# bjack205/rsLQR

Measured on AMD Instinct MI355X. Metric: LQR solves/sec (nx=12,nu=4,N=256,batch=1024 per GPU), higher is better.
Workload: dtype f64; 1 GPU; nx=12 nu=4 N=256 batch=1024 per GPU, fp64, factor+solve per step; parallelism=batch-sharded x1, no data-path collective, ranks_seen=1, flags=0, schedule=reduced-fused2

## Files before the change

### include/ndlqr_hip.h

```cpp
#ifndef NDLQR_HIP_H_
#define NDLQR_HIP_H_

#include <stddef.h>
#include <stdint.h>

#ifdef __cplusplus
extern "C" {
#endif

typedef struct NdlqrHipCtx NdlqrHipCtx;

int ndlqr_hip_device_count(void);
const char* ndlqr_hip_last_error(void);

NdlqrHipCtx* ndlqr_hip_create(int nstates, int ninputs, int nhorizon, int batch, int device);
#define NDLQR_CREATE_NO_PAD 1u
NdlqrHipCtx* ndlqr_hip_create_ex(int nstates, int ninputs, int nhorizon, int batch, int device, unsigned create_flags);
void ndlqr_hip_destroy(NdlqrHipCtx* ctx);
int ndlqr_hip_set_flags(NdlqrHipCtx* ctx, unsigned flags);
unsigned ndlqr_hip_get_flags(const NdlqrHipCtx* ctx);
int ndlqr_hip_set_stream(NdlqrHipCtx* ctx, void* hip_stream);
void* ndlqr_hip_get_stream(NdlqrHipCtx* ctx);

int ndlqr_hip_upload_inputs(NdlqrHipCtx* ctx, int p0, int count, const double* AB,
// ... 114 lines not shown
void ndlqr_hip_device_free(void* p);
int ndlqr_hip_copy(void* dst, const void* src, size_t bytes);

int ndlqr_hip_download_solutions(NdlqrHipCtx* ctx, int p0, int count, double* soln);
int ndlqr_hip_download_rhs_blocks(NdlqrHipCtx* ctx, int p, double* z_full);
int ndlqr_hip_download_factors(NdlqrHipCtx* ctx, int p, double* fact);
int ndlqr_hip_factors_valid(const NdlqrHipCtx* ctx);
int ndlqr_hip_pack_solutions_device(NdlqrHipCtx* ctx, double* dst);
int ndlqr_hip_kkt_residual(NdlqrHipCtx* ctx, double* res, double* bnorm);
int ndlqr_hip_cholesky_failures(NdlqrHipCtx* ctx);
int ndlqr_hip_download_failure_counts(NdlqrHipCtx* ctx, int* counts);
const char* ndlqr_hip_schedule(const NdlqrHipCtx* ctx);
int ndlqr_hip_compact_level1(const NdlqrHipCtx* ctx);
int ndlqr_hip_level1_paired(const NdlqrHipCtx* ctx);
int ndlqr_hip_bottom_lds16(const NdlqrHipCtx* ctx);

int ndlqr_hip_profile_slots(NdlqrHipCtx* ctx);
int ndlqr_hip_profile_get(NdlqrHipCtx* ctx, int slot, char* name, int name_cap, double* total_ms,
                          int* launches);
int ndlqr_hip_profile_reset(NdlqrHipCtx* ctx);

int ndlqr_hip_gemm(int tA, int tB, int m, int n, int k, double alpha, const double* A, int lda,
                   const double* B, int ldb, double beta, double* C, int ldc);
int ndlqr_hip_potrf_lower(int n, double* A, int lda);
int ndlqr_hip_potrs_lower(int n, int nrhs, const double* L, int ldl, double* B, int ldb);
int ndlqr_hip_trsv_lower(int n, int nrhs, const double* L, int ldl, double* B, int ldb, int transposed);

#ifdef __cplusplus
}
#endif
// ... 2 lines not shown
```

### rslqr_amd/__init__.py

```python
from .api import (
    BOUNDS_SHARED,
    BatchSolver,
    DeviceArray,
    FLAG_GENERIC,
    FLAG_KEEP_FACT,
    FLAG_KEEP_RECORDS,
    FLAG_PROFILE,
    FLAG_STRICT_FP,
    GRAD_A,
    GRAD_B,
    GRAD_DENSE_NAMES,
    GRAD_NAMES,
    GRAD_Q,
    GRAD_R,
    GRAD_d,
    GRAD_q,
    GRAD_r,
    GRAD_x0,
    GRADD_A,
    GRADD_B,
    GRADD_H,
    GRADD_Q,
    GRADD_R,
    GRADD_d,
# ... 8 lines not shown
    NdLqrBoxSettings,
    NdLqrBoxSettingsFull,
    NdLqrSolver,
    SOLN_INPUT,
    SOLN_ONLY,
    SOLN_LAMBDA,
    SOLN_STATE,
    device_count,
    exported_symbols,
    feedback_gains_lds,
    generate_synthetic,
    lib,
    library_path,
    objective_constants,
    pinned_empty,
)
```

### rslqr_amd/api.py

```python
import ctypes as C
import os
import re

import numpy as np

from . import build as _build

FLAG_STRICT_FP = 1
FLAG_GENERIC = 2
FLAG_PROFILE = 4
FLAG_KEEP_FACT = 8
FLAG_KEEP_RECORDS = 16
SOLN_LAMBDA, SOLN_STATE, SOLN_INPUT, SOLN_ONLY = 1, 2, 4, 8
GRAD_A, GRAD_B, GRAD_Q, GRAD_R, GRAD_q, GRAD_r, GRAD_d, GRAD_x0 = 1, 2, 4, 8, 16, 32, 64, 128
GRAD_NAMES = ("A", "B", "Q", "R", "q", "r", "d", "x0")
GRADD_A, GRADD_B, GRADD_Q, GRADD_H, GRADD_R, GRADD_q, GRADD_r, GRADD_d, GRADD_x0 = 1, 2, 4, 8, 16, 32, 64, 128, 256
GRAD_DENSE_NAMES = ("A", "B", "Q", "H", "R", "q", "r", "d", "x0")

ERR_INVALID = -1
ERR_NO_DEVICE = -2
ERR_NOT_SPD = -3

dp = C.POINTER(C.c_double)

# ... 308 lines not shown
    proto("ndlqr_hip_profile_slots", ci, vp)
    proto("ndlqr_hip_profile_get", ci, vp, ci, C.c_char_p, ci, dp, C.POINTER(ci))
    proto("ndlqr_hip_profile_reset", ci, vp)
    proto("ndlqr_hip_device_pointers", ci, vp, C.POINTER(vp))
    proto("ndlqr_hip_staged_io", ci, vp, C.POINTER(dp), C.POINTER(dp), C.POINTER(dp), C.POINTER(dp))
    proto("ndlqr_hip_download_rhs_blocks", ci, vp, ci, dp)
    proto("ndlqr_hip_upload_inputs", ci, vp, ci, ci, dp, dp, dp)
    proto("ndlqr_hip_factors_valid", ci, vp)
    proto("ndlqr_hip_schedule", C.c_char_p, vp)
    if hasattr(L, "ndlqr_hip_compact_level1"):
        proto("ndlqr_hip_compact_level1", C.c_int, vp)
    if hasattr(L, "ndlqr_hip_level1_paired"):
        proto("ndlqr_hip_level1_paired", C.c_int, vp)
    if hasattr(L, "ndlqr_hip_bottom_lds16"):
        proto("ndlqr_hip_bottom_lds16", C.c_int, vp)
    proto("ndlqr_hip_set_pipeline_depth", ci, vp, ci)
    proto("ndlqr_hip_pipeline_depth", ci, vp)
    proto("ndlqr_hip_pack_solutions_device", ci, vp, vp)
    proto("ndlqr_hip_gemm", ci, ci, ci, ci, ci, ci, cd, dp, ci, dp, ci, cd, dp, ci)
    proto("ndlqr_hip_potrf_lower", ci, ci, dp, ci)
    proto("ndlqr_hip_potrs_lower", ci, ci, ci, dp, ci, dp, ci)
    proto("ndlqr_hip_trsv_lower", ci, ci, ci, dp, ci, dp, ci, ci)
    _LIB = L
    return L


def pinned_empty(shape):
    import weakref
    count = int(np.prod(shape))
    L = lib()
# ... 110 lines not shown
        if not hasattr(a, "ptr"):
            if a.shape not in ((k,), (N, k), (B, N, k)):
                raise ValueError("bounds of shape %s: expected (%d,), (%d, %d) or (%d, %d, %d)" % (a.shape, k, N, k, B, N, k))
            a = np.ascontiguousarray(np.broadcast_to(a, (N, k) if shared else (B, N, k)))
            keep.append(a)
        ptrs.append(_any_ptr(a, (1 if shared else B) * N * k))
    return ptrs, shared, keep


def generate_synthetic(n, m, N, seed):
    out = dict(A=np.zeros((N, n * n)), B=np.zeros((N, n * m)), Q=np.zeros((N, n)),
               R=np.zeros((N, m)), q=np.zeros((N, n)), r=np.zeros((N, m)), d=np.zeros((N, n)),
               x0=np.zeros(n))
    _call(lib(), "ndlqr_GenerateSyntheticFlat", n, m, N, seed, *[_ptr(a) for a in out.values()], detail=False)
    return out


class BatchSolver:

    def __init__(self, n, m, N, batch, device=-1, flags=0):
        self.L = lib()
        self.n, self.m, self.N, self.batch = n, m, N, batch
        self.h = self.L.ndlqr_NewBatchSolver(n, m, N, batch, device)
        if not self.h:
            raise RuntimeError("ndlqr_NewBatchSolver failed: %s" %
                               self.L.ndlqr_hip_last_error().decode())
        self.nvars = self.L.ndlqr_BatchNumVars(self.h)
        self._sel = None
        self._step_refs = []
        self._rows = 0
# ... 589 lines not shown
```

### rslqr_amd/csrc/hip_context.hpp

```cpp
#pragma once
#include <hip/hip_runtime.h>

#include <cstdio>
#include <cstdlib>
#include <cstring>
#include <initializer_list>
#include <string>
#include <utility>
#include <vector>

#include "ndlqr.h"
#include "ndlqr_hip.h"

#include "kernels_common.hpp"

#pragma GCC visibility push(hidden)
int ndlqr_hip_fail(const char* what, hipError_t e);
struct NdlqrHipCtx;
int ndlqr_hip_ensure_F(NdlqrHipCtx* c);
#pragma GCC visibility pop
#define HIP_TRY(expr)                                                  \
  do {                                                                 \
    hipError_t e_ = (expr);                                            \
    if (e_ != hipSuccess) return ndlqr_hip_fail(#expr, e_);            \
// ... 15 lines not shown
  hipEvent_t start, stop;
};

enum class Family { None, Small, GenericReduced, GenericKnot };

struct KeptState {
  Family family = Family::None;
  bool time_shard = false;
  bool rec_complete = false;
  bool rec_compact = false;
  bool fact_valid = false;
  const char* schedule = "none";
  bool rec1_compact = false;
  bool level1_paired = false;
  bool bottom_lds16 = false;
  void forget_factorisation() { rec_complete = fact_valid = false; }
};

struct CapturedChain {
  hipGraphExec_t exec = nullptr;
  unsigned flags = 0;
  hipStream_t stream = nullptr;
  unsigned apply = 0;
  void reset() {
    if (exec) (void)hipGraphExecDestroy(exec);
    exec = nullptr;
  }
};

struct KnotSlice {
// ... 75 lines not shown
  unsigned long long rhs_gen[4] = {};
  CapturedChain graph;
  bool ready = false;
  hipError_t ensure_xfer(const ndlqr::Dims& u) { return xfer.ensure((size_t)u.batch * u.N * u.rows + (size_t)u.batch * u.n); }
};


struct DevKnobs {
  int rowbcast = -1;
  int tree = -1;
  int backsub_cols = -1;
  int fuse2 = -1;
  int compact1 = -1;
  int pair1 = -1;
  int bottom_lds16 = -1;
  int pipeline = 2;
  bool no_top = false;
  int top_levels = 3;
  bool no_mfma = false;
  int sep_threads = 0;
  int mult_threads = 0;
  bool no_reduced_generic = false;
  bool no_pad = false;
  bool alt_priority_set = false;
  int alt_priority = 0;
};

struct AdjointState {
  DevBuf<double> rhs, z;
  DevBuf<double> save;
  unsigned long long gen = 0;
  unsigned long long rhs_stamp = 0;
// ... 342 lines not shown
```

### rslqr_amd/csrc/kernels_bottom_reduced.hpp

```cpp
#pragma once
#include "kernels_dpp.hpp"
#include "kernels_small.hpp"

namespace ndlqr {

typedef double acc4_t __attribute__((ext_vector_type(4)));

template <int NX>
struct McPitch {
  static constexpr int SP = 18, WP = 17;
};

template <int NX, class Hook>
__device__ __forceinline__ void factor_tail_mc(const int lane, const acc4_t& c, const double (&ra)[(NX + 3) / 4],
                                               const double (&rb)[(NX + 3) / 4], const double* Wm, acc4_t& X0,
                                               acc4_t& X1, Hook hook) {
  constexpr int KS = (NX + 3) / 4, WP = McPitch<NX>::WP;
  int lane_o = lane;
  asm volatile("" : "+v"(lane_o));
  const int li = lane_o & 15, lk = lane_o >> 4;
  double wt[KS], wa[KS], b0[KS];
#pragma unroll
  for (int q = 0; q < KS; ++q) {
    wt[q] = Wm[(4 * q + lk) * WP + li];
// ... 867 lines not shown
      flag_failure(info, d, b);
  }
  __syncthreads();
  pair1_tail_park_mc<NX, NU>(d, kw + 4 * wave, b, lane, lds[wave].buf, hd, wave == 0, mslot, park);
  __syncthreads();
  asm volatile("" : "+v"(lane));
  if (wave == 0) reduced_eliminate_pass_mc<NX, NU>(d, kw, b, lane, c_m, mslot, info, lds[0].buf);
  __syncthreads();
  if (wave == 0) reduced_eliminate_gram_park_mc<NX, NU>(d, kw, b, lane, red, lds[0].buf, park);
  else reduced_eliminate_tail_mc<NX, NU>(d, kw, b, lane, false, red, rec, lds[0].buf);
}

template <int NX>
__device__ __forceinline__ void backsub_top_body(const Dims& d, const int b, const int t,
                                                 const double* __restrict__ recs, double* __restrict__ ytop,
                                                 double* ytop_lds, const int bp = -1, const double* zsep = nullptr);
template <int NX, int NU>
__global__ __launch_bounds__(256) __attribute__((amdgpu_waves_per_eu(4))) void reduced_top_mc(Dims d, const int l0, const double* __restrict__ AB,
                                                      const double* __restrict__ QR, const double* __restrict__ rhs,
                                                      double* red, double* __restrict__ rec, double* F,
                                                      int* __restrict__ info, const int store_l,
                                                      double* __restrict__ ytop) {
  __shared__ ReducedLds<NX, NU, false> lds[4];
  const int wave = __builtin_amdgcn_readfirstlane(threadIdx.x >> 6), b = blockIdx.x;
  for (int l = l0, s0 = 0; l < d.K;) {
    int lane = threadIdx.x & 63;
    asm volatile("" : "+v"(lane));
    const int cnt = d.N >> (l + 1);
    if (wave + s0 < cnt)
      reduced_separator_mc<NX, NU, true>(d, l, (wave + s0) * (2 << l), b, lane, AB, QR, rhs, red, rec, F, info, store_l,
                                         lds[wave]);
// ... 296 lines not shown
```

### rslqr_amd/csrc/kernels_rowbcast.hpp

```cpp
#pragma once
#include "kernels_dpp.hpp"
#include "kernels_small.hpp"

namespace ndlqr {

template <int K, bool NEG>
__device__ __forceinline__ void fmac_bc4(double& a0, double& a1, double& a2, double& a3, const double x0, const double x1,
                                         const double x2, const double x3, const double y) {
  if constexpr (NEG)
    asm volatile("v_fmac_f64_dpp %0, -%4, %8 row_newbcast:%9 row_mask:0xf bank_mask:0xf\n\t"
                 "v_fmac_f64_dpp %1, -%5, %8 row_newbcast:%9 row_mask:0xf bank_mask:0xf\n\t"
                 "v_fmac_f64_dpp %2, -%6, %8 row_newbcast:%9 row_mask:0xf bank_mask:0xf\n\t"
                 "v_fmac_f64_dpp %3, -%7, %8 row_newbcast:%9 row_mask:0xf bank_mask:0xf"
                 : "+v"(a0), "+v"(a1), "+v"(a2), "+v"(a3) : "v"(x0), "v"(x1), "v"(x2), "v"(x3), "v"(y), "n"(K));
  else
    asm volatile("v_fmac_f64_dpp %0, %4, %8 row_newbcast:%9 row_mask:0xf bank_mask:0xf\n\t"
                 "v_fmac_f64_dpp %1, %5, %8 row_newbcast:%9 row_mask:0xf bank_mask:0xf\n\t"
                 "v_fmac_f64_dpp %2, %6, %8 row_newbcast:%9 row_mask:0xf bank_mask:0xf\n\t"
                 "v_fmac_f64_dpp %3, %7, %8 row_newbcast:%9 row_mask:0xf bank_mask:0xf"
                 : "+v"(a0), "+v"(a1), "+v"(a2), "+v"(a3) : "v"(x0), "v"(x1), "v"(x2), "v"(x3), "v"(y), "n"(K));
}

template <int KD, int NC, bool INIT, bool NEG = false, int NA, int NB>
__device__ __forceinline__ void rb_mul(const double (&A)[NA], double (&B)[NB], double (&out)[NC]) {
// ... 338 lines not shown
    }
    rb_mul<NX, NX, true>(RbTt, Xb, G);
    gv = rb_mulv<NX>(RbTt, xz);
    if (hasB && rowlane) {
#pragma unroll
      for (int c = 0; c < NX; ++c)
        if (c >= i) atomicAdd(sB.DL() + c * (c + 1) / 2 + i, G[c]);
      atomicAdd(sB.gL() + i, gv);
    }
  }
}

template <int NX>
__device__ __forceinline__ void backsub_top_body(const Dims& d, const int b, const int t,
                                                 const double* __restrict__ recs, double* __restrict__ ytop,
                                                 double* ytop_lds, const int bp, const double* zsep) {
  constexpr int NN = NX * NX, REC = 2 * NN + NX;
  const int N = d.N, K = d.K;
  const int br = bp >= 0 ? bp : b;
  for (int L = K - 1; L >= 3; --L) {
    const int T = 2 << L, nsep = N >> (L + 1);
    for (int it = t; it < nsep * NX; it += 256) {
      const int q = it / NX, r = it - q * NX;
      const int base = q * T, s = base + (T >> 1) - 1;
      const double* rc = recs + ((size_t)br * N + s) * REC;
      double acc = zsep ? zsep[((size_t)b * N + s) * NX + r] : rc[2 * NN + r];
      if (base > 0) {
        double f[NX];
        load_row<NX>(rc + r * NX, f);
        const double* y = ytop_lds + ((base - 1) >> 3) * NX;
#pragma unroll
        for (int c = 0; c < NX; ++c) acc = fma(-f[c], y[c], acc);
      }
      if (base + T < N) {
        double f[NX];
        load_row<NX>(rc + NN + r * NX, f);
        const double* y = ytop_lds + ((base + T - 1) >> 3) * NX;
#pragma unroll
        for (int c = 0; c < NX; ++c) acc = fma(-f[c], y[c], acc);
      }
      ytop_lds[(s >> 3) * NX + r] = acc;
    }
    __syncthreads();
  }
  double* out = ytop + (size_t)b * (N >> 3) * NX;
  for (int e = t; e < ((N >> 3) - 1) * NX; e += 256) out[e] = ytop_lds[e];
}

template <int NX>
__global__ __launch_bounds__(256) void rb_backsub_top(Dims d, const double* __restrict__ recs, double* __restrict__ ytop) {
  extern __shared__ double ytop_lds[];
  backsub_top_body<NX>(d, blockIdx.x, threadIdx.x, recs, ytop, ytop_lds);
}

template <int NX, int NU>
struct alignas(16) RbBacksubLds {
  static constexpr int W = NX + NU, ROWS = 2 * NX + NU, NN = NX * NX, REC = 2 * NN + NX, R0 = NX * (NX + 1) / 2;
  static constexpr int R0P = (R0 + 1) / 2 * 2;
  static constexpr int WP = RbKnot<NX, NU>::WP;
  double ab[8][NX * WP];
  double rec0[4][R0P];
// ... 799 lines not shown
```

### rslqr_amd/csrc/launch_small.hpp

```cpp
#pragma once
#include "hip_context.hpp"
#include "kernels_leaf.hpp"
#include "kernels_small.hpp"
#include "kernels_bottom_reduced.hpp"
#include "kernels_rowbcast.hpp"

constexpr int kBottomLevels = 2;

struct SmallPlan {
  bool strict, keep;
  bool lean;
  int store_l;
  bool reduced;
  bool tree;
  bool compact;
  bool rowbcast;
  bool fuse2;
  bool compact1;
  bool pair1;
  bool lds16;
  int level0;
  int ltop;
  int top_l0;
  bool top_sweeps;
  size_t top_lds;
  const char* schedule;
  bool rec_complete, rec_compact;
  bool needs_F;
};

template <int NX, int NU>
constexpr bool kRbBacksubFits = 8 * (2 * NX + NU) <= 256;

static inline unsigned apply_grid(const NdlqrHipCtx* c, const ndlqr::Dims& d) {
  return (unsigned)(c->apply_nblk > 0 ? c->apply_nblk : d.N / 8);
}
static inline ndlqr::Dims apply_dims(const NdlqrHipCtx* c, const ndlqr::Dims& d) {
  ndlqr::Dims da = d;
  if (c->apply_nblk > 0) da.xoff += c->apply_blk0;
  return da;
}

template <int NX, int NU>
constexpr bool kCompact1Fits = ndlqr::P1OnMatrixCores<NX, NU>::value && NX >= 9 && NX + NU <= 16;

template <int NX, int NU>
constexpr bool kPair1Fits = kCompact1Fits<NX, NU> && ndlqr::McPair1Layout<NX>::SIZE <= ndlqr::ReducedLds<NX, NU>::NBUF;

template <int NX, int NU, bool MULTI, class... Args>
static void launch_rb_backsub(const NdlqrHipCtx* c, const dim3 grid, hipStream_t stream, const bool compact1,
                              const Args&... args) {
  if constexpr (NX + NU <= 16) {
    if constexpr (kCompact1Fits<NX, NU> && !MULTI) {
      if (compact1) {
        hipLaunchKernelGGL((ndlqr::rb_backsub<NX, NU, false, true, true>), grid, dim3(ndlqr::kRbBacksubColsThreads), 0, stream,
                           args...);
        return;
      }
    }
    if (c->knobs.backsub_cols != 0) {
      hipLaunchKernelGGL((ndlqr::rb_backsub<NX, NU, MULTI, true>), grid, dim3(ndlqr::kRbBacksubColsThreads), 0, stream, args...);
      return;
// ... 27 lines not shown
      p.compact1 = kCompact1Fits<NX, NU> && p.compact && !p.store_l && !p.rowbcast && c->knobs.backsub_cols != 0 &&
                   (c->knobs.compact1 > 0 ||
                    (c->knobs.compact1 < 0 && ((NX == 12 && NU == 4 && p.fuse2) || (NX == 10 && NU == 4))));
      p.pair1 = kPair1Fits<NX, NU> && p.fuse2 && p.compact1 &&
                (c->knobs.pair1 > 0 || (c->knobs.pair1 < 0 && NX == 12 && NU == 4));
      p.lds16 = p.pair1 && c->knobs.bottom_lds16 != 0;
      p.schedule = p.tree ? "reduced-tree"
                   : !p.compact ? "reduced-records"
                   : p.store_l ? "reduced-compact-records" : (p.fuse2 ? "reduced-fused2" : "reduced");
      if (!p.tree) {
        const int top_levels = d.K - c->knobs.top_levels >= 3 ? c->knobs.top_levels : 3;
        p.level0 = p.fuse2 ? 3 : 2;
        p.ltop = (d.K >= 5 && !c->knobs.no_top) ? d.K - top_levels : d.K;
        p.top_l0 = (p.fuse2 && p.ltop < 3) ? 3 : p.ltop;
        p.top_sweeps = p.ltop < d.K && p.compact && p.top_lds <= 4 * sizeof(ndlqr::ReducedLds<NX, NU, false>);
      }
    }
  }
  p.needs_F = !(p.reduced && p.store_l != 1);
  return p;
}

template <int NX, int NU, bool STRICT, bool KEEP>
static int launch_small(NdlqrHipCtx* c, const SmallPlan& plan) {
  const ndlqr::Dims& d = c->d;
  BufferSet& s = c->set[c->cur];
  using Sh = ndlqr::SchurShape<NX, NU>;
  constexpr int JB = kBottomLevels;
  const bool lean = plan.lean;
  const int store_l = plan.store_l;
// ... 40 lines not shown
              done = true;
            }
          }
          if (!done)
            hipLaunchKernelGGL((ndlqr::bottom_reduced_mc<NX, NU, false, true>), dim3(d.N >> 2, d.batch), dim3(64), 0, s.stream,
                               d, c->AB, c->QR, s.rhs, s.red, s.rec, c->F, c->info, store_l, nullptr, 1);
        } else
          hipLaunchKernelGGL((ndlqr::bottom_reduced_mc<NX, NU, false>), dim3(d.N >> 2, d.batch), dim3(64), 0, s.stream,
                             d, c->AB, c->QR, s.rhs, s.red, s.rec, c->F, c->info, store_l, nullptr, 0);
      }
      for (int l = plan.level0; l < plan.ltop; ++l) {
        ScopedSlot t(c, SLOT_UPPER);
        hipLaunchKernelGGL((ndlqr::reduced_level_mc<NX, NU>), dim3(d.N >> (l + 1), d.batch), dim3(64), 0, s.stream,
                           d, l, c->AB, c->QR, s.rhs, s.red, s.rec, c->F, c->info, store_l);
      }
      if (plan.ltop < d.K) {
        ScopedSlot t(c, SLOT_TOP);
        hipLaunchKernelGGL((ndlqr::reduced_top_mc<NX, NU>), dim3(d.batch), dim3(256), 0, s.stream, d, plan.top_l0, c->AB,
                           c->QR, s.rhs, s.red, s.rec, c->F, c->info, store_l, plan.top_sweeps ? s.ytop : (double*)nullptr);
      }
      ScopedSlot t(c, SLOT_APPLY);
      if (plan.compact) {
        if (!plan.top_sweeps) {
          (void)allow_dynamic_lds(&ndlqr::rb_backsub_top<NX>, plan.top_lds);
          hipLaunchKernelGGL((ndlqr::rb_backsub_top<NX>), dim3(d.batch), dim3(256), plan.top_lds, s.stream, d, s.rec, s.ytop);
        }
        launch_rb_backsub<NX, NU, false>(c, dim3(apply_grid(c, d), d.batch), s.stream, plan.compact1,
                           apply_dims(c, d), c->AB, c->QR, s.rhs, s.rec, s.ytop, s.z);
      } else {
        hipLaunchKernelGGL((ndlqr::backsub_small<NX, NU>), dim3(apply_grid(c, d), d.batch), dim3(256), 0, s.stream, apply_dims(c, d), c->AB,
                           c->QR, s.rhs, s.rec, s.z);
// ... 176 lines not shown
```

### rslqr_amd/csrc/ndlqr_hip.hip

```cpp
#include "hip_host.hpp"
#include "kernels_generic.hpp"
#include "kernels_mfma.hpp"
#include "launch_reduced.hpp"
#include "kernels_reduced_solve.hpp"
#include "launch_small.hpp"


static thread_local std::string g_last_error = "";

const char* ndlqr_hip_last_error(void) { return g_last_error.c_str(); }

int ndlqr_hip_fail(const char* what, hipError_t e) {
  g_last_error = std::string(what) + ": " + hipGetErrorString(e);
  fprintf(stderr, "ndlqr_hip: %s\n", g_last_error.c_str());
  if (e == hipErrorInvalidConfiguration || e == hipErrorInvalidValue) return NDLQR_ERR_INVALID;
  return NDLQR_ERR_NO_DEVICE;
}
int fail(const char* what, hipError_t e) { return ndlqr_hip_fail(what, e); }
int refuse(const std::string& msg) {
  g_last_error = msg;
  fprintf(stderr, "ndlqr_hip: %s\n", g_last_error.c_str());
  return NDLQR_ERR_INVALID;
}

// ... 62 lines not shown
static size_t bytes_z(const ndlqr::Dims& d) { return sizeof(double) * doubles_z(d); }
static size_t bytes_F(const ndlqr::Dims& d) { return sizeof(double) * doubles_F(d); }

static DevKnobs read_knobs() {
  DevKnobs k;
  const auto num = [](const char* name, int* v) { if (getenv(name)) *v = atoi(getenv(name)); };
  const auto onoff = [](const char* name, int* v) { if (getenv(name)) *v = atoi(getenv(name)) != 0 ? 1 : 0; };
  num("NDLQR_PIPELINE", &k.pipeline);
  onoff("NDLQR_TREE", &k.tree);
  onoff("NDLQR_ROWBCAST", &k.rowbcast);
  onoff("NDLQR_FUSE2", &k.fuse2);
  onoff("NDLQR_BACKSUB_COLS", &k.backsub_cols);
  onoff("NDLQR_COMPACT1", &k.compact1);
  onoff("NDLQR_PAIR1", &k.pair1);
  onoff("NDLQR_BOTTOM_LDS16", &k.bottom_lds16);
  k.no_mfma = getenv("NDLQR_NO_MFMA") != nullptr;
  k.no_top = getenv("NDLQR_NO_TOP") != nullptr;
  num("NDLQR_TOP_LEVELS", &k.top_levels);
  if (k.top_levels < 3 || k.top_levels > 5) k.top_levels = 3;
  num("NDLQR_SEP_THREADS", &k.sep_threads);
  num("NDLQR_MULT_THREADS", &k.mult_threads);
  k.no_reduced_generic = getenv("NDLQR_DEV_NO_REDUCED_GENERIC") != nullptr;
  k.no_pad = getenv("NDLQR_NO_PAD") != nullptr;
  k.alt_priority_set = getenv("NDLQR_ALT_PRIORITY") != nullptr;
  num("NDLQR_ALT_PRIORITY", &k.alt_priority);
  return k;
}

static bool alloc_set(NdlqrHipCtx* c, BufferSet& s, bool slots) {
  const ndlqr::Dims& d = c->d;
  hipError_t e = first_error({hipEventCreate(&s.ev_start), hipEventCreate(&s.ev_stop), s.rec.ensure((size_t)d.batch * d.N * (2 * d.n * d.n + d.n)),
                              s.rhs.ensure(doubles_z(d)), s.h_fail.ensure_zeroed(1)});
// ... 577 lines not shown
  const ndlqr::Dims& d = c->d;
  SolvePlan p = {};
  p.strict = (c->flags & NDLQR_FLAG_STRICT_FP) != 0;
  p.keep = (c->flags & NDLQR_FLAG_KEEP_FACT) != 0;
  p.inst = pick_small(c);
  if (p.inst) {
    p.family = Family::Small;
    p.small = p.inst->plan(c, p.strict, p.keep);
    p.needs_F = p.small.needs_F;
    p.kept.schedule = p.small.schedule;
    p.kept.rec_complete = p.small.rec_complete;
    p.kept.rec_compact = p.small.rec_compact;
    p.kept.rec1_compact = p.small.compact1;
    p.kept.level1_paired = p.small.pair1;
    p.kept.bottom_lds16 = p.small.lds16;
  } else if ((p.red = plan_reduced_generic(c)).ok) {
    p.family = Family::GenericReduced;
    p.needs_red_generic = true;
    p.kept.schedule = p.red.keep ? "generic-reduced-records" : "generic-reduced";
    p.kept.rec_complete = p.red.keep;
  } else {
    p.family = Family::GenericKnot;
    p.rec_as_factors = (c->flags & NDLQR_FLAG_KEEP_RECORDS) && !p.strict;
    p.lean = !p.strict && !p.keep && !p.rec_as_factors;
    p.needs_F = true;
    p.sep = plan_generic_sep(c, p.strict);
    if (p.sep.scratch)
      p.sep_scratch_bytes = sizeof(double) * ((size_t)d.n * (d.n + 1) + (size_t)d.n * (2 * d.n + 1)) * (size_t)d.batch *
                            (d.N / 2 > 0 ? d.N / 2 : 1);
    p.kept.schedule = p.lean ? "generic-lean" : (p.strict ? "generic-strict" : "generic-keep");
// ... 915 lines not shown
      if (e == hipSuccess) memcpy(soln + off, c->h_stage[(i - 1) & 1], sizeof(double) * len);
    }
  }
  c->event_pool.push_back(done[0]);
  c->event_pool.push_back(done[1]);
  if (e != hipSuccess) return fail("ndlqr_hip_download_solutions", e);
  return NDLQR_OK;
}

const char* ndlqr_hip_schedule(const NdlqrHipCtx* c) { return c ? c->kept.schedule : "none"; }

int ndlqr_hip_compact_level1(const NdlqrHipCtx* c) { return c && c->kept.rec1_compact ? 1 : 0; }

int ndlqr_hip_level1_paired(const NdlqrHipCtx* c) { return c && c->kept.level1_paired ? 1 : 0; }
int ndlqr_hip_bottom_lds16(const NdlqrHipCtx* c) { return c && c->kept.bottom_lds16 ? 1 : 0; }

int ndlqr_hip_factors_valid(const NdlqrHipCtx* c) { return c && c->kept.fact_valid ? 1 : 0; }

int ndlqr_hip_pack_solutions_device(NdlqrHipCtx* c, double* dst) {
  if (!c || !dst) return NDLQR_ERR_INVALID;
  if (c->z_partial || c->z_invalid) return need_full_solution(c, "ndlqr_hip_pack_solutions_device");
  const ndlqr::Dims& d = c->d;
  HIP_TRY(hipSetDevice(c->device));
  HIP_TRY(launch_pack(c->du, d, KnotSlice(), c->set[c->latest].z, dst, c->set[c->latest].stream, d.batch));
  if (c->cost.dense && !c->cost.mapped(c->soln_gen)) HIP_TRY(cost_map_back(c, dst, 0, d.batch, c->set[c->latest].stream));
  return NDLQR_OK;
}

int ndlqr_hip_kkt_residual(NdlqrHipCtx* c, double* res, double* bnorm) {
  if (!c || !res) return NDLQR_ERR_INVALID;
// ... 97 lines not shown
```

### rslqr_amd/roofline.py

```python
import math

HBM_PEAK_GBS = 8000.0
FP64_PEAK_TFLOPS = 78.6


def record_doubles(n, level, compact_level0=False, compact_level1=False):
    if (compact_level0 and level == 0) or (compact_level1 and level == 1):
        return n * (n + 1) // 2
    return 2 * n * n + n


def separator_flops(n, w):
    leaf = 2 * n * n * w + 2 * n * w
    chol = n ** 3 / 3.0
    solves = 2 * n * n * (2 * n + 1)
    schur = 4 * n ** 3 + 4 * n * n
    return leaf + chol + solves + schur


def backsub_flops(n, m, N):
    w = n + m
    return (N - 1) * 4 * n * n + N * (2 * n * w + 3 * (2 * n + m))


# ... 51 lines not shown
    if K > 2:
        out["upper"] = {"bytes": 8 * upper_b, "flops": nsep_upper * fs, "launches": K - 2}
    if K >= 5 and compact_level0:
        per_sep = upper_b // nsep_upper
        sweep_b = (N // 8 - 1) * rec + (N // 8) * n
        sweep_f = (N // 8 - 1) * 4 * n * n
        out["top"] = {"bytes": 8 * (7 * per_sep + sweep_b), "flops": 7 * fs + sweep_f, "launches": 1}
        out["upper"] = {"bytes": 8 * (nsep_upper - 7) * per_sep, "flops": (nsep_upper - 7) * fs, "launches": K - 5}
        out["apply"] = {"bytes": out["apply"]["bytes"] - 8 * sweep_b, "flops": out["apply"]["flops"] - sweep_f,
                        "launches": 1}
        if nsep_upper == 7:
            del out["upper"]
    return out


def knot_lean_model(n, m, N):
    K = int(math.log2(N))
    w, rows = n + m, 2 * n + m
    fb = rows * n
    rec = 2 * n * n + n
    fs = separator_flops(n, w)
    bottom_b = inputs_doubles(n, m, N) + (3 * N // 4) * rec + (N // 2) * (2 * fb + rows)
    out = {"bottom": {"bytes": 8 * bottom_b, "flops": (3 * N // 4) * fs + N * 4 * fb * n, "launches": 1},
           "apply": {"bytes": 8 * ((N - 1) * rec + inputs_doubles(n, m, N) + N * rows),
                     "flops": backsub_flops(n, m, N), "launches": 1}}
    if K > 2:
        nsep = N // 4 - 1
        per = (2 * w * n + 2 * n * n + rows + 2 * n + n * w) + rec + 2 * (3 * fb + 2 * rows)
        out["upper"] = {"bytes": 8 * nsep * per, "flops": nsep * (fs + 2 * 4 * fb * n), "launches": K - 2}
    return out
# ... 33 lines not shown
    sep_b = 0
    for l in range(K):
        L = N >> (l + 1)
        own = n * w + (w + n) + (rows + 2 * n)
        if l == 0:
            sep_b += L * (own + n * n + rec0 + push)
        else:
            sep_b += L * (own + slot + rec0 + push + (2 * sym + 2 * n))
    return {
        "separator": {"bytes": 8 * sep_b, "flops": (N - 1) * separator_flops(n, w), "launches": K},
        "apply": {"bytes": 8 * ((N - 1) * rec0 + (N // 2 - 1) * 2 * n * n + inputs_doubles(n, m, N) + N * rows),
                  "flops": backsub_flops(n, m, N) + (N - 1) * 2 * n * n, "launches": 1},
    }


def model_for(schedule, n, m, N, compact1=False):
    if schedule == "reduced":
        return reduced_model(n, m, N, compact_level0=True, compact_level1=compact1)
    if schedule == "reduced-fused2":
        return reduced_model(n, m, N, compact_level0=True, fused2=True, compact_level1=compact1)
    if schedule in ("reduced-tree", "reduced-records"):
        return reduced_model(n, m, N)
    if schedule == "knot-lean":
        return knot_lean_model(n, m, N)
    if schedule == "generic-lean":
        return generic_lean_model(n, m, N)
    if schedule in ("generic-reduced", "generic-reduced-records"):
        return generic_reduced_model(n, m, N)
    return None


def model_b_bytes(n, m, N):
    K = int(math.log2(N))
    Fb = (2 * n + m) * n
    total = N * (4 * n * n + 3 * m * n + m * m + 5 * n + 3 * m)
# ... 38 lines not shown
```

Measured before the change: 2.081 million solves/s.

## Replace top-level tree reduction with two-ended chain elimination kernel

Adds a reduced_chain_top kernel that handles the top five levels of the separator tree. Instead of reducing them level by level, it eliminates the separators as a sequential chain from both ends, with two waves meeting in the middle and handing off through LDS. The same kernel runs the back-substitution sweep into ytop. This cuts per-level launches and synchronisation, and packs four batch elements per 128-thread block. In exchange, work that was parallel becomes a serial chain of dependent steps. The path is on by default only when K=8 and (nx,nu) is one of a hardcoded list of measured sizes, which includes 12/4.

```diff
diff --git a/include/ndlqr_hip.h b/include/ndlqr_hip.h
--- a/include/ndlqr_hip.h
+++ b/include/ndlqr_hip.h
@@ -152,6 +152,7 @@
 int ndlqr_hip_compact_level1(const NdlqrHipCtx* ctx);
 int ndlqr_hip_level1_paired(const NdlqrHipCtx* ctx);
 int ndlqr_hip_bottom_lds16(const NdlqrHipCtx* ctx);
+int ndlqr_hip_top_chain(const NdlqrHipCtx* ctx);
 
 int ndlqr_hip_profile_slots(NdlqrHipCtx* ctx);
 int ndlqr_hip_profile_get(NdlqrHipCtx* ctx, int slot, char* name, int name_cap, double* total_ms,
diff --git a/rslqr_amd/__init__.py b/rslqr_amd/__init__.py
--- a/rslqr_amd/__init__.py
+++ b/rslqr_amd/__init__.py
@@ -46,4 +46,5 @@
     library_path,
     objective_constants,
     pinned_empty,
+    top_chain,
 )
diff --git a/rslqr_amd/api.py b/rslqr_amd/api.py
--- a/rslqr_amd/api.py
+++ b/rslqr_amd/api.py
@@ -346,6 +346,8 @@
         proto("ndlqr_hip_level1_paired", C.c_int, vp)
     if hasattr(L, "ndlqr_hip_bottom_lds16"):
         proto("ndlqr_hip_bottom_lds16", C.c_int, vp)
+    if hasattr(L, "ndlqr_hip_top_chain"):
+        proto("ndlqr_hip_top_chain", C.c_int, vp)
     proto("ndlqr_hip_set_pipeline_depth", ci, vp, ci)
     proto("ndlqr_hip_pipeline_depth", ci, vp)
     proto("ndlqr_hip_pack_solutions_device", ci, vp, vp)
@@ -486,6 +488,10 @@
                x0=np.zeros(n))
     _call(lib(), "ndlqr_GenerateSyntheticFlat", n, m, N, seed, *[_ptr(a) for a in out.values()], detail=False)
     return out
+
+
+def top_chain(solver):
+    return hasattr(solver.L, "ndlqr_hip_top_chain") and bool(solver.L.ndlqr_hip_top_chain(solver.ctx))
 
 
 class BatchSolver:
diff --git a/rslqr_amd/csrc/hip_context.hpp b/rslqr_amd/csrc/hip_context.hpp
--- a/rslqr_amd/csrc/hip_context.hpp
+++ b/rslqr_amd/csrc/hip_context.hpp
@@ -53,6 +53,7 @@
   bool rec1_compact = false;
   bool level1_paired = false;
   bool bottom_lds16 = false;
+  bool top_chain = false;
   void forget_factorisation() { rec_complete = fact_valid = false; }
 };
 
@@ -158,8 +159,10 @@
   int compact1 = -1;
   int pair1 = -1;
   int bottom_lds16 = -1;
+  int top_chain = -1;
   int pipeline = 2;
   bool no_top = false;
+  bool top_levels_set = false;
   int top_levels = 3;
   bool no_mfma = false;
   int sep_threads = 0;
diff --git a/rslqr_amd/csrc/kernels_bottom_reduced.hpp b/rslqr_amd/csrc/kernels_bottom_reduced.hpp
--- a/rslqr_amd/csrc/kernels_bottom_reduced.hpp
+++ b/rslqr_amd/csrc/kernels_bottom_reduced.hpp
@@ -905,7 +905,8 @@
 template <int NX>
 __device__ __forceinline__ void backsub_top_body(const Dims& d, const int b, const int t,
                                                  const double* __restrict__ recs, double* __restrict__ ytop,
-                                                 double* ytop_lds, const int bp = -1, const double* zsep = nullptr);
+                                                 double* ytop_lds, const int bp = -1, const double* zsep = nullptr,
+                                                 const int ltop = 0, const int nt = 256);
 template <int NX, int NU>
 __global__ __launch_bounds__(256) __attribute__((amdgpu_waves_per_eu(4))) void reduced_top_mc(Dims d, const int l0, const double* __restrict__ AB,
                                                       const double* __restrict__ QR, const double* __restrict__ rhs,
diff --git a/rslqr_amd/csrc/kernels_chain_top.hpp b/rslqr_amd/csrc/kernels_chain_top.hpp
--- /dev/null
+++ b/rslqr_amd/csrc/kernels_chain_top.hpp
@@ -0,0 +1,265 @@
+#pragma once
+#include "kernels_bottom_reduced.hpp"
+#include "kernels_rowbcast.hpp"
+
+namespace ndlqr {
+
+template <int NX, int NU>
+constexpr bool kChainTopFits = NX + 1 <= 16 && NU <= 16;
+template <int NX, int NU>
+constexpr bool kChainTopSplit = NX + NU > 16;
+
+constexpr int kChainTopThreads = 128;
+constexpr int kChainTopMaxLevels = 5;
+
+template <int NX>
+struct alignas(16) ChainTopLds {
+  double hand[4][NX + 1][16];
+  double lmid[4][NX][NX + 1];
+  double ymid[4][16];
+};
+
+template <int NX, int NU>
+struct ChainOps {
+  double abrow[NX + NU];
+  double tcol[NX];
+  double tcolb[kChainTopSplit<NX, NU> ? NX : 1];
+  double qkb, zkb;
+  double dl[NX], dr[NX];
+  double cpl[NX];
+  double qk, zk;
+  double q1, z1l, z1x;
+  double gl, gr;
+};
+
+template <int NX, int NU>
+__device__ __forceinline__ void chain_load(const Dims& d, const int l0, const int b, const int j, const int dir, const int ic,
+                                           const int kc, const double* __restrict__ AB, const double* __restrict__ QR,
+                                           const double* __restrict__ rhs, const double* red, ChainOps<NX, NU>& o) {
+  constexpr int W = NX + NU, ROWS = 2 * NX + NU, NN = NX * NX, TRI = RedSlot<NX>::TRI, SLOT = RedSlot<NX>::SIZE;
+  const int N = d.N, s = ((j + 1) << l0) - 1;
+  const size_t kn = (size_t)b * N + s;
+  const double* abm = AB + kn * NX * W;
+#pragma unroll
+  for (int k = 0; k < W; ++k) o.abrow[k] = abm[ic * W + k];
+#pragma unroll
+  for (int c = 0; c < NX; ++c) o.tcol[c] = abm[c * W + kc];
+  o.qk = QR[kn * W + kc];
+  o.zk = rhs[kn * ROWS + NX + kc];
+  if constexpr (kChainTopSplit<NX, NU>) {
+    const int kb = NX + (kc < NU ? kc : NU - 1);
+#pragma unroll
+    for (int c = 0; c < NX; ++c) o.tcolb[c] = abm[c * W + kb];
+    o.qkb = QR[kn * W + kb];
+    o.zkb = rhs[kn * ROWS + NX + kb];
+  }
+  o.q1 = QR[(kn + 1) * W + ic];
+  o.z1l = rhs[(kn + 1) * ROWS + ic];
+  o.z1x = rhs[(kn + 1) * ROWS + NX + ic];
+  const double* sl = red + ((size_t)b * (N >> 2) + (s >> 2)) * SLOT;
+#pragma unroll
+  for (int c = 0; c < NX; ++c) {
+    const int tix = RedSlot<NX>::tri(ic, c);
+    o.dl[c] = sl[tix];
+    o.dr[c] = sl[TRI + tix];
+  }
+  o.gl = sl[2 * TRI + 2 * NN + ic];
+  o.gr = sl[2 * TRI + 2 * NN + NX + ic];
+  if (dir != 0) {
+    const bool own = (j & 1) == 0;
+    const int sn = own ? s : s + dir * (1 << l0);
+    const double* cs = red + ((size_t)b * (N >> 2) + (sn >> 2)) * SLOT + 2 * TRI + (((dir > 0) == own) ? NN : 0);
+    const double* cp = cs + (own ? ic : ic * NX);
+    const int sk = own ? NX : 1;
+#pragma unroll
+    for (int k = 0; k < NX; ++k) o.cpl[k] = cp[k * sk];
+  } else {
+#pragma unroll
+    for (int k = 0; k < NX; ++k) o.cpl[k] = 0.0;
+  }
+}
+
+template <int NX, int NU>
+__device__ __forceinline__ void chain_assemble(const int i, ChainOps<NX, NU>& o, const double (&U)[NX], const double ub,
+                                               double (&S)[NX], double& bz) {
+  constexpr int W = NX + NU;
+  const double wk = rb_rcp(o.qk);
+  double T[NX];
+#pragma unroll
+  for (int c = 0; c < NX; ++c) T[c] = o.tcol[c] * wk;
+  if constexpr (kChainTopSplit<NX, NU>) {
+    const double wb = rb_rcp(o.qkb), q1 = rb_rcp(o.q1);
+    double Tb[NX], brow[NU];
+#pragma unroll
+    for (int c = 0; c < NX; ++c) Tb[c] = o.tcolb[c] * wb;
+#pragma unroll
+    for (int k = 0; k < NU; ++k) brow[k] = o.abrow[NX + k];
+    rb_mul<NX, NX, true>(o.abrow, T, S);
+    rb_mul<NU, NX, false>(brow, Tb, S);
+    bz = rb_mulv<NU>(brow, o.zkb * wb, rb_mulv<NX>(o.abrow, o.zk * wk)) - fma(o.z1x, q1, o.z1l);
+#pragma unroll
+    for (int c = 0; c < NX; ++c) S[c] += (c == i) ? q1 : 0.0;
+  } else {
+    rb_leaf<NX, W>(i, o.abrow, T, o.zk * wk, rb_rcp(o.q1), o.z1l, o.z1x, S, bz);
+  }
+#pragma unroll
+  for (int c = 0; c < NX; ++c) S[c] = (S[c] - (o.dl[c] + o.dr[c])) + U[c];
+  bz = (bz - (o.gl + o.gr)) + ub;
+}
+
+template <int NX, int NU>
+__global__ __launch_bounds__(kChainTopThreads) void reduced_chain_top(Dims d, const int l0, const double* __restrict__ AB,
+                                                                      const double* __restrict__ QR,
+                                                                      const double* __restrict__ rhs, const double* red,
+                                                                      double* rec, int* __restrict__ info,
+                                                                      double* __restrict__ ytop) {
+  static_assert(kChainTopFits<NX, NU>, "panel and leaf tile fit a DPP row");
+  constexpr int NN = NX * NX, REC = 2 * NN + NX;
+  extern __shared__ double chain_ys[];
+  __shared__ ChainTopLds<NX> lds;
+  const int N = d.N, K = d.K;
+  const int wave = __builtin_amdgcn_readfirstlane((int)threadIdx.x >> 6), lane = threadIdx.x & 63;
+  const int r = lane >> 4, i = lane & 15;
+  const int ic = i < NX ? i : NX - 1;
+  const int kc = kChainTopSplit<NX, NU> ? (i < 16 ? i : 15) : (i < NX + NU ? i : NX + NU - 1);
+  const int bm = 4 * (int)blockIdx.x + r;
+  const bool valid = bm < d.batch;
+  const int b = valid ? bm : d.batch - 1;
+  const int C = (1 << (K - l0)) - 1, mid = C >> 1;
+  const int dir = wave ? -1 : 1;
+  double* const ys = chain_ys + (size_t)r * (N >> 3) * NX;
+  auto sep_of = [&](const int j) { return ((j + 1) << l0) - 1; };
+
+  double U[NX], ub = 0.0;
+#pragma unroll
+  for (int c = 0; c < NX; ++c) U[c] = 0.0;
+  ChainOps<NX, NU> o;
+  if (mid > 0) chain_load<NX, NU>(d, l0, b, wave ? C - 1 : 0, dir, ic, kc, AB, QR, rhs, red, o);
+  for (int step = 0; step < mid; ++step) {
+    const int j = wave ? C - 1 - step : step;
+    double S[NX], w[NX], bz;
+    chain_assemble<NX, NU>(i, o, U, ub, S, bz);
+    dpp_fence(bz);
+    sfor<NX>([&](auto kk) {
+      constexpr int k = decltype(kk)::value;
+      const double bk = row_bc<k>(bz);
+      w[k] = (i == NX) ? bk : -o.cpl[k];
+    });
+    const int jn = j + dir;
+    chain_load<NX, NU>(d, l0, b, jn, jn == mid ? 0 : dir, ic, kc, AB, QR, rhs, red, o);
+    if (rb_chol_inv<NX, false>(i, S, w) && i == 0 && valid) {
+      atomicAdd(info + b, K - l0);
+      atomicAdd(info + d.batch, K - l0);
+    }
+    if (valid) {
+      double* const sc = rec + ((size_t)b * N + sep_of(j)) * REC;
+      if (i < NX) {
+#pragma unroll
+        for (int k = 0; k < NX; ++k) sc[k * NX + i] = w[k];
+        store_row<NX>(sc + NN + i * NX, S);
+      } else if (i == NX) {
+#pragma unroll
+        for (int k = 0; k < NX; ++k) sc[2 * NN + k] = w[k];
+      }
+    }
+#pragma unroll
+    for (int c = 0; c < NX; ++c) U[c] = 0.0;
+    ub = 0.0;
+    dpp_fence(w);
+    sfor<NX>([&](auto kk) {
+      constexpr int k = decltype(kk)::value;
+      sfor<NX>([&](auto cc) {
+        constexpr int c = decltype(cc)::value;
+        fnmac_bc<c>(U[c], w[k], w[k]);
+      });
+      fnmac_bc<NX>(ub, w[k], w[k]);
+    });
+  }
+  if (mid == 0 && wave == 0) chain_load<NX, NU>(d, l0, b, 0, 0, ic, kc, AB, QR, rhs, red, o);
+
+  if (wave == 1) {
+#pragma unroll
+    for (int c = 0; c < NX; ++c) lds.hand[r][c][i] = U[c];
+    lds.hand[r][NX][i] = ub;
+  }
+  asm volatile("s_waitcnt vmcnt(0)" ::: "memory");
+  __syncthreads();
+  double ynext;
+  if (wave == 0) {
+    double S[NX], w[NX], bz;
+#pragma unroll
+    for (int c = 0; c < NX; ++c) U[c] += lds.hand[r][c][i];
+    ub += lds.hand[r][NX][i];
+    chain_assemble<NX, NU>(i, o, U, ub, S, bz);
+    if (rb_chol_inv<NX>(i, S, w) && i == 0 && valid) {
+      atomicAdd(info + b, K - l0);
+      atomicAdd(info + d.batch, K - l0);
+    }
+    if (i < NX) {
+#pragma unroll
+      for (int c = 0; c < NX; ++c) lds.lmid[r][i][c] = S[c];
+    }
+    wave_lds_sync();
+    double lrow[NX], lcol[NX];
+#pragma unroll
+    for (int c = 0; c < NX; ++c) {
+      const double up = lds.lmid[r][c][ic];
+      lrow[c] = (c < i && i < NX) ? S[c] : 0.0;
+      lcol[c] = (c > i && i < NX) ? up : 0.0;
+    }
+    const double dinv = rb_rcp(lds.lmid[r][ic][ic]);
+    ynext = rb_llt_solve<NX>(bz, lrow, lcol, dinv);
+    lds.ymid[r][i] = ynext;
+    if (i < NX) ys[(sep_of(mid) >> 3) * NX + i] = ynext;
+  }
+  __syncthreads();
+  if (wave == 1) ynext = lds.ymid[r][i];
+
+  struct Back { double yrow[NX], lcol[NX], ld, v; };
+  auto back_load = [&](const int j, Back& k) {
+    const double* sc = rec + ((size_t)b * N + sep_of(j)) * REC;
+#pragma unroll
+    for (int c = 0; c < NX; ++c) k.yrow[c] = sc[ic * NX + c];
+#pragma unroll
+    for (int e = 0; e < NX; ++e) k.lcol[e] = sc[NN + e * NX + ic];
+    k.ld = sc[NN + ic * NX + ic];
+    k.v = sc[2 * NN + ic];
+  };
+  Back cur;
+  if (mid > 0) back_load(wave ? mid + 1 : mid - 1, cur);
+  for (int step = mid - 1; step >= 0; --step) {
+    const int j = wave ? C - 1 - step : step;
+    Back nxt;
+    back_load(step > 0 ? j - dir : j, nxt);
+    double x0 = cur.v, x1 = 0.0;
+    dpp_fence(ynext);
+    sfor<NX>([&](auto cc) {
+      constexpr int c = decltype(cc)::value;
+      if constexpr (c % 2 == 0) fnmac_bc<c>(x0, ynext, cur.yrow[c]);
+      else fnmac_bc<c>(x1, ynext, cur.yrow[c]);
+    });
+    const double dinv = rb_rcp(cur.ld);
+    double lc[NX];
+#pragma unroll
+    for (int e = 0; e < NX; ++e) lc[e] = (e > i && i < NX) ? cur.lcol[e] * dinv : 0.0;
+    double x = (x0 + x1) * dinv;
+    sfor<NX - 1>([&](auto cc) {
+      constexpr int e = NX - 1 - decltype(cc)::value;
+      dpp_fence(x);
+      fnmac_bc<e>(x, x, lc[e]);
+    });
+    ynext = x;
+    if (i < NX) ys[(sep_of(j) >> 3) * NX + i] = x;
+    cur = nxt;
+  }
+  __syncthreads();
+
+  for (int q = 0; q < 4; ++q) {
+    const int bq = 4 * (int)blockIdx.x + q;
+    if (bq < d.batch)
+      backsub_top_body<NX>(d, bq, threadIdx.x, rec, ytop, chain_ys + (size_t)q * (N >> 3) * NX, -1, nullptr, l0,
+                           kChainTopThreads);
+  }
+}
+
+}
diff --git a/rslqr_amd/csrc/kernels_rowbcast.hpp b/rslqr_amd/csrc/kernels_rowbcast.hpp
--- a/rslqr_amd/csrc/kernels_rowbcast.hpp
+++ b/rslqr_amd/csrc/kernels_rowbcast.hpp
@@ -376,13 +376,14 @@
 template <int NX>
 __device__ __forceinline__ void backsub_top_body(const Dims& d, const int b, const int t,
                                                  const double* __restrict__ recs, double* __restrict__ ytop,
-                                                 double* ytop_lds, const int bp, const double* zsep) {
+                                                 double* ytop_lds, const int bp, const double* zsep, const int ltop,
+                                                 const int nt) {
   constexpr int NN = NX * NX, REC = 2 * NN + NX;
   const int N = d.N, K = d.K;
   const int br = bp >= 0 ? bp : b;
-  for (int L = K - 1; L >= 3; --L) {
+  for (int L = (ltop > 0 ? ltop : K) - 1; L >= 3; --L) {
     const int T = 2 << L, nsep = N >> (L + 1);
-    for (int it = t; it < nsep * NX; it += 256) {
+    for (int it = t; it < nsep * NX; it += nt) {
       const int q = it / NX, r = it - q * NX;
       const int base = q * T, s = base + (T >> 1) - 1;
       const double* rc = recs + ((size_t)br * N + s) * REC;
@@ -406,7 +407,7 @@
     __syncthreads();
   }
   double* out = ytop + (size_t)b * (N >> 3) * NX;
-  for (int e = t; e < ((N >> 3) - 1) * NX; e += 256) out[e] = ytop_lds[e];
+  for (int e = t; e < ((N >> 3) - 1) * NX; e += nt) out[e] = ytop_lds[e];
 }
 
 template <int NX>
diff --git a/rslqr_amd/csrc/launch_small.hpp b/rslqr_amd/csrc/launch_small.hpp
--- a/rslqr_amd/csrc/launch_small.hpp
+++ b/rslqr_amd/csrc/launch_small.hpp
@@ -4,6 +4,7 @@
 #include "kernels_small.hpp"
 #include "kernels_bottom_reduced.hpp"
 #include "kernels_rowbcast.hpp"
+#include "kernels_chain_top.hpp"
 
 constexpr int kBottomLevels = 2;
 
@@ -22,6 +23,7 @@
   int level0;
   int ltop;
   int top_l0;
+  bool chain;
   bool top_sweeps;
   size_t top_lds;
   const char* schedule;
@@ -46,6 +48,10 @@
 
 template <int NX, int NU>
 constexpr bool kPair1Fits = kCompact1Fits<NX, NU> && ndlqr::McPair1Layout<NX>::SIZE <= ndlqr::ReducedLds<NX, NU>::NBUF;
+
+template <int NX, int NU>
+constexpr bool kChainTopMeasured = (NX == 12 && NU == 4) || (NX == 10 && NU == 4) || (NX == 9 && NU == 3) ||
+                                   (NX == 8 && NU == 4) || (NX == 6 && NU == 3) || (NX == 13 && NU == 4);
 
 template <int NX, int NU, bool MULTI, class... Args>
 static void launch_rb_backsub(const NdlqrHipCtx* c, const dim3 grid, hipStream_t stream, const bool compact1,
@@ -103,6 +109,15 @@
         p.ltop = (d.K >= 5 && !c->knobs.no_top) ? d.K - top_levels : d.K;
         p.top_l0 = (p.fuse2 && p.ltop < 3) ? 3 : p.ltop;
         p.top_sweeps = p.ltop < d.K && p.compact && p.top_lds <= 4 * sizeof(ndlqr::ReducedLds<NX, NU, false>);
+        if constexpr (ndlqr::kChainTopFits<NX, NU>) {
+          p.chain = p.compact && !p.store_l && d.K >= 4 && !c->knobs.no_top && !c->knobs.top_levels_set &&
+                    sizeof(ndlqr::ChainTopLds<NX>) + 4 * p.top_lds <= kLdsMax &&
+                    (c->knobs.top_chain > 0 || (c->knobs.top_chain < 0 && d.K == 8 && kChainTopMeasured<NX, NU>));
+          if (p.chain) {
+            p.ltop = p.top_l0 = d.K - ndlqr::kChainTopMaxLevels > 3 ? d.K - ndlqr::kChainTopMaxLevels : 3;
+            p.top_sweeps = true;
+          }
+        }
       }
     }
   }
@@ -173,7 +188,18 @@
         hipLaunchKernelGGL((ndlqr::reduced_level_mc<NX, NU>), dim3(d.N >> (l + 1), d.batch), dim3(64), 0, s.stream,
                            d, l, c->AB, c->QR, s.rhs, s.red, s.rec, c->F, c->info, store_l);
       }
-      if (plan.ltop < d.K) {
+      bool chained = false;
+      if constexpr (ndlqr::kChainTopFits<NX, NU>) {
+        if (plan.chain) {
+          ScopedSlot t(c, SLOT_TOP);
+          const size_t lds = 4 * plan.top_lds;
+          (void)allow_dynamic_lds(&ndlqr::reduced_chain_top<NX, NU>, lds);
+          hipLaunchKernelGGL((ndlqr::reduced_chain_top<NX, NU>), dim3((d.batch + 3) / 4), dim3(ndlqr::kChainTopThreads), lds,
+                             s.stream, d, plan.ltop, c->AB, c->QR, s.rhs, s.red, s.rec, c->info, s.ytop);
+          chained = true;
+        }
+      }
+      if (!chained && plan.ltop < d.K) {
         ScopedSlot t(c, SLOT_TOP);
         hipLaunchKernelGGL((ndlqr::reduced_top_mc<NX, NU>), dim3(d.batch), dim3(256), 0, s.stream, d, plan.top_l0, c->AB,
                            c->QR, s.rhs, s.red, s.rec, c->F, c->info, store_l, plan.top_sweeps ? s.ytop : (double*)nullptr);
diff --git a/rslqr_amd/csrc/ndlqr_hip.hip b/rslqr_amd/csrc/ndlqr_hip.hip
--- a/rslqr_amd/csrc/ndlqr_hip.hip
+++ b/rslqr_amd/csrc/ndlqr_hip.hip
@@ -100,8 +100,10 @@
   onoff("NDLQR_COMPACT1", &k.compact1);
   onoff("NDLQR_PAIR1", &k.pair1);
   onoff("NDLQR_BOTTOM_LDS16", &k.bottom_lds16);
+  onoff("NDLQR_TOP_CHAIN", &k.top_chain);
   k.no_mfma = getenv("NDLQR_NO_MFMA") != nullptr;
   k.no_top = getenv("NDLQR_NO_TOP") != nullptr;
+  k.top_levels_set = getenv("NDLQR_TOP_LEVELS") != nullptr;
   num("NDLQR_TOP_LEVELS", &k.top_levels);
   if (k.top_levels < 3 || k.top_levels > 5) k.top_levels = 3;
   num("NDLQR_SEP_THREADS", &k.sep_threads);
@@ -709,6 +711,7 @@
     p.kept.rec1_compact = p.small.compact1;
     p.kept.level1_paired = p.small.pair1;
     p.kept.bottom_lds16 = p.small.lds16;
+    p.kept.top_chain = p.small.chain;
   } else if ((p.red = plan_reduced_generic(c)).ok) {
     p.family = Family::GenericReduced;
     p.needs_red_generic = true;
@@ -1654,6 +1657,7 @@
 
 int ndlqr_hip_level1_paired(const NdlqrHipCtx* c) { return c && c->kept.level1_paired ? 1 : 0; }
 int ndlqr_hip_bottom_lds16(const NdlqrHipCtx* c) { return c && c->kept.bottom_lds16 ? 1 : 0; }
+int ndlqr_hip_top_chain(const NdlqrHipCtx* c) { return c && c->kept.top_chain ? 1 : 0; }
 
 int ndlqr_hip_factors_valid(const NdlqrHipCtx* c) { return c && c->kept.fact_valid ? 1 : 0; }
 
diff --git a/rslqr_amd/roofline.py b/rslqr_amd/roofline.py
--- a/rslqr_amd/roofline.py
+++ b/rslqr_amd/roofline.py
@@ -89,6 +89,41 @@
     return out
 
 
+def chain_block_flops(n, w):
+    leaf = 2 * n * n * w + 2 * n * w
+    return leaf + n ** 3 / 3.0 + n * n * (n + 1) + 2 * n * n * (n + 1) + 2 * n * n + n * n
+
+
+def chain_top_model(base, n, m, N, fused2):
+    K = int(math.log2(N))
+    if K < 4:
+        return base
+    w, rows = n + m, 2 * n + m
+    tri = n * (n + 1) // 2
+    rec = record_doubles(n, 2)
+    l0 = max(3, K - 5)
+    blocks = (1 << (K - l0)) - 1
+    slot = 2 * tri + 2 * n * n + 2 * n
+    push = 2 * tri + n * n + 2 * n
+    per_sep = slot + n * w + w + n + rows + 2 * n + rec + push
+    per_block = (2 * tri + n * n + 2 * n) + n * w + w + n + rows + 2 * n + 2 * rec
+    level0 = 3 if fused2 else 2
+    left = sum(N >> (l + 1) for l in range(level0, l0))
+    swept = sum(N >> (l + 1) for l in range(3, l0))
+    out = dict(base)
+    if "top" not in out:
+        sweep_b = (N // 8 - 1) * rec + (N // 8) * n
+        out["apply"] = {"bytes": out["apply"]["bytes"] - 8 * sweep_b, "flops": out["apply"]["flops"] - (N // 8 - 1) * 4 * n * n,
+                        "launches": 1}
+    out["top"] = {"bytes": 8 * (blocks * per_block + swept * rec + (N // 8) * n),
+                  "flops": blocks * chain_block_flops(n, w) + swept * 4 * n * n, "launches": 1}
+    if left > 0:
+        out["upper"] = {"bytes": 8 * left * per_sep, "flops": left * separator_flops(n, w), "launches": l0 - level0}
+    else:
+        out.pop("upper", None)
+    return out
+
+
 def knot_lean_model(n, m, N):
     K = int(math.log2(N))
     w, rows = n + m, 2 * n + m
@@ -152,11 +187,13 @@
     }
 
 
-def model_for(schedule, n, m, N, compact1=False):
+def model_for(schedule, n, m, N, compact1=False, chain=False):
     if schedule == "reduced":
-        return reduced_model(n, m, N, compact_level0=True, compact_level1=compact1)
+        base = reduced_model(n, m, N, compact_level0=True, compact_level1=compact1)
+        return chain_top_model(base, n, m, N, False) if chain else base
     if schedule == "reduced-fused2":
-        return reduced_model(n, m, N, compact_level0=True, fused2=True, compact_level1=compact1)
+        base = reduced_model(n, m, N, compact_level0=True, fused2=True, compact_level1=compact1)
+        return chain_top_model(base, n, m, N, True) if chain else base
     if schedule in ("reduced-tree", "reduced-records"):
         return reduced_model(n, m, N)
     if schedule == "knot-lean":
```

Result: faster. 2.210 million solves/s (median of 6 runs) (+6.2%).
